# NingZhang1/pyscf_isdf

Measured on AMD Instinct MI355X. Metric: isdf_build_plus_get_jk_wall_time, lower is better.
Workload: dtype f64

## Files before the change

### include/mi355_isdf.h

```cpp
#ifndef MI355_ISDF_H
#define MI355_ISDF_H

#include <stdint.h>

#ifdef __cplusplus
extern "C" {
#endif

typedef struct isdf_ctx* isdf_handle;

#define ISDF_OK 0
#define ISDF_ERR_ARG 1
#define ISDF_ERR_HIP 2
#define ISDF_ERR_LIB 3
#define ISDF_ERR_NUM 4

int isdf_abi_version(void);

int isdf_create(int device_id, isdf_handle* out);
int isdf_destroy(isdf_handle h);
int isdf_set_stream(isdf_handle h, void* hip_stream);
const char* isdf_last_error(isdf_handle h);
int64_t isdf_workspace_bytes(isdf_handle h);
int isdf_release_workspace(isdf_handle h);
// ... 42 lines not shown

int isdf_select_ip(isdf_handle h, const double* d_ao, int nao, int64_t ld,
                   int nblk, const int64_t* blk_off, const int32_t* nip,
                   double tol, double tie_rtol,
                   double* d_L, int64_t ldL, int64_t* d_piv, int32_t* rank);

int isdf_select_ip_ws(isdf_handle h, const double* d_ao, int nao, int64_t ld,
                      int nblk, const int64_t* blk_off, const int32_t* nip,
                      double tol, double tie_rtol,
                      double* d_L, int64_t ldL, int64_t* d_piv, int32_t* rank,
                      void* d_work, int64_t work_bytes);
int64_t isdf_select_ip_work_bytes(int nao, int64_t m);

int isdf_select_ip_gram(isdf_handle h, double* d_A, int m, int64_t ldA, int nip, double tol, double tie_rtol,
                        int panel, int64_t* d_piv, int32_t* rank);

int isdf_select_ip_cplx(isdf_handle h, const double* d_ao, int nao, int nh, int64_t ld,
                        int nblk, const int64_t* blk_off, const int32_t* nip,
                        double tol, double tie_rtol,
                        double* d_L, int64_t ldL, int64_t* d_piv, int32_t* rank);

int isdf_fit_from_chol(isdf_handle h, double* d_L, int k, int64_t m, int64_t ldL,
                       const int64_t* d_piv);

int isdf_fit_prepare(isdf_handle h, const double* d_ao, int nao, int64_t ld,
                     const int64_t* d_ip, int P, double reg_rel, double* d_aoP, double* d_chol,
                     double* reg_used);
int isdf_fit_apply(isdf_handle h, const double* d_chol, const double* d_aoP, int P, int nao,
                   const double* d_ao, int64_t ng, int64_t ld, int forward_only,
                   double* d_theta, int64_t ldt);
int isdf_fit_prepare_cplx(isdf_handle h, const double* d_ao, int nao, int nh, int64_t ld,
                          const int64_t* d_ip, int P, double reg_rel, double* d_aoP, double* d_chol,
                          double* reg_used);
int isdf_fit_apply_cplx(isdf_handle h, const double* d_chol, const double* d_aoP, int P, int nao, int nh,
                        const double* d_ao, int64_t ng, int64_t ld, int forward_only,
                        double* d_theta, int64_t ldt);
int isdf_fit_global(isdf_handle h, const double* d_ao, int nao, int64_t ngrids, int64_t ld,
                    const int64_t* d_ip, int P, double reg_rel, double* d_theta, int64_t ldt,
                    double* d_aoP, double* reg_used);

int isdf_gather_aoP(isdf_handle h, const double* d_ao, int nao, int64_t ld, const int64_t* d_ip, int P,
                    double* d_aoP);
int isdf_gram_sq(isdf_handle h, const double* d_aoP, int P, int nao, int nh, double* d_A);
int isdf_pair_gram_rows(isdf_handle h, const double* d_aoP, int P, int nao, int nh, const double* d_ao,
                        int64_t ng, int64_t ld, double* d_B, int64_t ldb);
int isdf_block_chol(isdf_handle h, const double* d_A, int P, int nblk, const int32_t* blk_off,
                    double shift_rel, double* d_D, double* shift_used);
int isdf_block_solve(isdf_handle h, const double* d_D, int P, int nblk, const int32_t* blk_off, int side,
                     int trans, double* d_X, int64_t n, int64_t ldx);
int isdf_block_invert(isdf_handle h, const double* d_D, int P, int nblk, const int32_t* blk_off, double* d_Dinv);
int isdf_block_apply(isdf_handle h, const double* d_Dinv, int64_t ldd, int nblk, const int32_t* blk_off,
                     double* d_X, int64_t n, int64_t ldx);
int isdf_pair_rows_block_apply(isdf_handle h, const double* d_aoP, int P, int nao, const double* d_ao, int64_t ng,
                               int64_t ld, const double* d_Dinv, int64_t ldd, int nblk, const int32_t* blk_off,
                               double* d_B, int64_t ldb);

int isdf_gram_prod(isdf_handle h, const double* d_aoP, int P, int nao, const double* d_psiP, int nocc, double* d_A);
int isdf_pair_prod_rows(isdf_handle h, const double* d_aoP, int P, int nao, const double* d_psiP, int nocc,
// ... 134 lines not shown
```

### pyscf_isdf_amd/backend.py

```python
import ctypes
import os
import numpy as np
import torch
from . import lib as _lib

_vp = ctypes.c_void_p


def _np_ptr(a):
    return a.ctypes.data_as(_vp)


class HipBackend:
    name = 'hip-gfx950'

    def __init__(self, device=0):
        if not torch.cuda.is_available():
            raise _lib.IsdfError('no GPU visible to torch; the ISDF path has no CPU fallback')
        self.device = torch.device('cuda', device)
        torch.cuda.set_device(self.device)
        self.handle = _lib.Handle(device)
        if os.environ.get('ISDF_TRSM') == 'subst':
            self.set_option('trsm_substitution', 1)
        if os.environ.get('ISDF_OWN_FFT') in ('0', '1', '2'):
# ... 175 lines not shown
        assert piv.dtype == torch.int64 and piv.is_contiguous() and ao.stride(1) == 1 and L.stride(1) == 1
        assert work is None or work.is_contiguous()
        self.handle.call('isdf_select_ip_ws', self._p(ao), ao.shape[0], ao.stride(0), len(nip), _np_ptr(blk_off),
                         _np_ptr(nip), float(tol), float(tie_rtol), self._p(L), L.stride(0), self._p(piv), _np_ptr(rank),
                         None if work is None else self._p(work), 0 if work is None else work.numel() * work.element_size())
        return rank

    def select_ip_gram(self, A, nip, tol, tie_rtol, piv, panel=0):
        self._stream()
        assert piv.dtype == torch.int64 and piv.is_contiguous() and A.stride(1) == 1 and A.shape[0] == A.shape[1]
        rank = ctypes.c_int32(0)
        self.handle.call('isdf_select_ip_gram', self._p(A), A.shape[0], A.stride(0), int(nip), float(tol), float(tie_rtol),
                         int(panel), self._p(piv), ctypes.byref(rank))
        return int(rank.value)

    def fit_from_chol(self, L, k, m, piv):
        self._stream()
        self.handle.call('isdf_fit_from_chol', self._p(L), int(k), int(m), L.stride(0), self._p(piv))

    def fit_prepare(self, ao, ip, reg_rel, aoP, chol):
        self._stream()
        assert ip.dtype == torch.int64 and aoP.is_contiguous() and chol.is_contiguous()
        reg = ctypes.c_double(0.0)
        self.handle.call('isdf_fit_prepare', self._p(ao), ao.shape[0], ao.stride(0), self._p(ip), ip.numel(),
                         float(reg_rel), self._p(aoP), self._p(chol), ctypes.byref(reg))
        return reg.value

    def fit_apply(self, chol, aoP, ao, ng, theta, forward_only=False):
        self._stream()
        self.handle.call('isdf_fit_apply', self._p(chol), self._p(aoP), aoP.shape[0], aoP.shape[1], self._p(ao),
                         int(ng), ao.stride(0), int(bool(forward_only)), self._p(theta), theta.stride(0))

    def gather_aoP(self, ao, ip, aoP):
        self._stream()
        self.handle.call('isdf_gather_aoP', self._p(ao), ao.shape[0], ao.stride(0), self._p(ip), ip.numel(), self._p(aoP))

    def gram_sq(self, aoP, A, nh=0):
        self._stream()
        self.handle.call('isdf_gram_sq', self._p(aoP), aoP.shape[0], aoP.shape[1], int(nh), self._p(A))

    def pair_gram_rows(self, aoP, ao, ng, B, nh=0):
        self._stream()
        self.handle.call('isdf_pair_gram_rows', self._p(aoP), aoP.shape[0], aoP.shape[1], int(nh), self._p(ao), int(ng),
                         ao.stride(0), self._p(B), B.stride(0))

    def gram_prod(self, aoP, psiP, A):
        self._stream()
        assert aoP.is_contiguous() and psiP.is_contiguous() and A.is_contiguous() and aoP.shape[0] == psiP.shape[0]
        self.handle.call('isdf_gram_prod', self._p(aoP), aoP.shape[0], aoP.shape[1], self._p(psiP), psiP.shape[1], self._p(A))

    def pair_prod_rows(self, aoP, psiP, ao, psi, ng, B):
        self._stream()
        assert aoP.is_contiguous() and psiP.is_contiguous() and aoP.shape[0] == psiP.shape[0]
# ... 471 lines not shown
```

### pyscf_isdf_amd/csrc/common.h

```cpp
#pragma once
#include <hip/hip_runtime.h>
#include <rocblas/rocblas.h>
#include <rocsolver/rocsolver.h>
#include <hipfft/hipfft.h>
#include <cstdint>
#include <cstdio>
#include <cstring>
#include <string>
#include <vector>
#include <map>
#include "../../include/mi355_isdf.h"

struct FftPlan {
  hipfftHandle fwd = 0, bwd = 0;
  size_t work_bytes = 0;
};

struct ProfRec {
  hipEvent_t e0 = nullptr, e1 = nullptr;
};
struct ProfEntry {
  std::vector<ProfRec> recs;
  double work = 0.0;
  double ms = 0.0;
// ... 9 lines not shown
};

struct isdf_ctx {
  int profiling = 0;
  std::map<std::string, ProfEntry> prof;
  int device = 0;
  hipStream_t stream = nullptr;
  rocblas_handle blas = nullptr;
  std::string err;
  std::map<std::vector<int>, FftPlan> plans;
  std::map<std::string, std::pair<void*, size_t>> ws;
  int num_cu = 256;
  int trsm_substitution = 0;
  int own_fft = 2;
  int gemm_nn_own = 0;
  int attr_gemm_b = 0, attr_gemm_nn = 0, attr_gram_tri = 0, attr_herm = 0;
  int cand_gram = 1;
  int conv_pipe = 1;
  int conv_sub_rows = 0;
  int gram_pivot_tpb = 256;
  int gram_compact = 1;
  int gram_compact_permille = 875;
  int block_apply_waves = 16;
  int block_apply_reg = 1;
  double coul_omega = 0.0;
  double coul_rc = 0.0;
  int coul_sphere = 0;
  WsKernel wsk;
};

int isdf_fail(isdf_handle h, int code, const char* fmt, ...);
void* isdf_ws(isdf_handle h, const char* name, size_t bytes);
int isdf_get_plan(isdf_handle h, const int32_t mesh[3], int batch, FftPlan** out);
int get_coulG_half(isdf_handle h, const int32_t mesh[3], const double a[9], double extra_scale, double** out);
bool conv_rows_own_supported(const int32_t mesh[3], int nb);
bool conv_rows_q_own_supported(isdf_handle h, const int32_t mesh[3], int nb);
bool spectral_rows_own_supported(isdf_handle h, const int32_t mesh[3], int nb);
// ... 71 lines not shown
                           int64_t ldb);
int gemm_nn_f64(isdf_handle h, int64_t M, int64_t N, int64_t K, const double* A, int64_t lda, const double* B, int64_t ldb,
                double* C, int64_t ldc, bool square);
int gemm_rm(isdf_handle h, char opA, char opB, int64_t M, int64_t N, int64_t K, double alpha,
            const double* A, int64_t lda, const double* B, int64_t ldb, double beta, double* C,
            int64_t ldc);

__host__ __device__ inline int64_t gram_tri_row(int64_t r) {
  const int64_t tm = r >> 8;
  return 32768 * tm * (tm + 1) + (r & 255) * ((tm + 1) << 8);
}
static inline int64_t gram_tri_size(int64_t m) { return m > 0 ? gram_tri_row(m - 1) + (((m - 1) >> 8) + 1) * 256 : 0; }
struct GramTriUnit { int blk, tm, tn, pad; };
int gram_tri_blocks(isdf_handle h, const double* X, int64_t ldx, int K, const GramTriUnit* d_units, int64_t nunits,
                    const int64_t* d_blk_off, int64_t row0, const int64_t* d_tri_off, double* S, double flop);
```

### pyscf_isdf_amd/csrc/fit.hip

```cpp
#include "common.h"
#include <cstdlib>

namespace {

__global__ void gather_T_kernel(const double* __restrict__ L, int64_t ldL,
                                const int64_t* __restrict__ piv, int k, double* __restrict__ T) {
  const int s = blockIdx.x * blockDim.x + threadIdx.x;
  const int t = blockIdx.y;
  if (s >= k) return;
  T[(int64_t)t * k + s] = (s >= t) ? L[(int64_t)t * ldL + piv[s]] : 0.0;
}

__global__ void square_kernel(double* __restrict__ x, int64_t rows, int64_t cols, int64_t ld) {
  const int64_t c = (int64_t)blockIdx.x * blockDim.x + threadIdx.x;
  const int64_t r = blockIdx.y;
  if (c >= cols) return;
  const double v = x[r * ld + c];
  x[r * ld + c] = v * v;
}

__global__ void square_add_kernel(double* __restrict__ x, int64_t ld, const double* __restrict__ y, int64_t ldy,
                                  int64_t cols) {
  const int64_t c = (int64_t)blockIdx.x * blockDim.x + threadIdx.x;
  const int64_t r = blockIdx.y;
// ... 217 lines not shown
  if (nh > 0) {
    double* rot = (double*)isdf_ws(h, "fit_rot", sizeof(double) * (size_t)P * nao);
    double* tmp = (double*)isdf_ws(h, "fit_tmp", sizeof(double) * (size_t)P * P);
    if (!rot || !tmp) return ISDF_ERR_HIP;
    hipLaunchKernelGGL(rotate_kernel, dim3((unsigned)cdiv(nao, 256), (unsigned)P), dim3(256), 0, h->stream, d_aoP, P, nh, rot);
    rc = gemm_rm(h, 'N', 'T', P, P, nao, 1.0, rot, nao, d_aoP, nao, 0.0, tmp, P);
    if (rc) return rc;
    hipLaunchKernelGGL(square_add_kernel, dim3((unsigned)cdiv(P, 256), (unsigned)P), dim3(256), 0, h->stream, d_A,
                       (int64_t)P, tmp, (int64_t)P, (int64_t)P);
  } else {
    hipLaunchKernelGGL(square_kernel, dim3((unsigned)cdiv(P, 256), (unsigned)P), dim3(256), 0, h->stream, d_A,
                       (int64_t)P, (int64_t)P, (int64_t)P);
  }
  KERNEL_CHECK(h);
  return ISDF_OK;
}

extern "C" int isdf_pair_gram_rows(isdf_handle h, const double* d_aoP, int P, int nao, int nh, const double* d_ao,
                                   int64_t ng, int64_t ld, double* d_B, int64_t ldb) {
  if (!h) return ISDF_ERR_ARG;
  ARG_CHECK(h, d_aoP && d_ao && d_B && P > 0 && P <= 65535 && nao > 0 && ng > 0 && ld >= ng && ldb >= ng);
  ARG_CHECK(h, nh == 0 || 2 * nh == nao);
  int rc = product_rows(h, P, ng, nao, d_aoP, d_ao, ld, d_B, ldb, nh == 0);
  if (rc) return rc;
  if (nh > 0) {
    const int64_t CH = 8192;
    double* rot = (double*)isdf_ws(h, "fit_rot", sizeof(double) * (size_t)P * nao);
    double* tmp = (double*)isdf_ws(h, "fit_tmpB", sizeof(double) * (size_t)P * CH);
    if (!rot || !tmp) return ISDF_ERR_HIP;
    hipLaunchKernelGGL(rotate_kernel, dim3((unsigned)cdiv(nao, 256), (unsigned)P), dim3(256), 0, h->stream, d_aoP, P, nh, rot);
// ... 414 lines not shown
```

### pyscf_isdf_amd/csrc/gemm_f64.hip

```cpp
#include "common.h"
#include <cstdlib>

int gemm_rm(isdf_handle h, char opA, char opB, int64_t M, int64_t N, int64_t K, double alpha,
            const double* A, int64_t lda, const double* B, int64_t ldb, double beta, double* C,
            int64_t ldc) {
  ARG_CHECK(h, M < 2147483647LL && N < 2147483647LL && K < 2147483647LL && lda < 2147483647LL &&
                   ldb < 2147483647LL && ldc < 2147483647LL);
  const rocblas_operation ta = (opA == 'N') ? rocblas_operation_none : rocblas_operation_transpose;
  const rocblas_operation tb = (opB == 'N') ? rocblas_operation_none : rocblas_operation_transpose;
  ProfScope ps(h, "rocblas_dgemm[flop]", 2.0 * M * N * (double)K);
  BLAS_TRY(h, rocblas_dgemm(h->blas, tb, ta, (rocblas_int)N, (rocblas_int)M, (rocblas_int)K, &alpha, B,
                            (rocblas_int)ldb, A, (rocblas_int)lda, &beta, C, (rocblas_int)ldc));
  return ISDF_OK;
}

namespace {

typedef double d4 __attribute__((ext_vector_type(4)));

constexpr int BM = 128, BN = 128, BK = 16;
constexpr int LDT = 17;
constexpr int TPB = 256;

struct GemmArgs {
// ... 166 lines not shown
  GemmArgs g;
  g.A = g.B = t.X + (r0 - t.row0) * t.ldx;
  g.lda = g.ldb = t.ldx;
  g.kscale = nullptr;
  g.M = g.N = (int)(t.blk_off[u.blk + 1] - r0);
  g.K = g.kslab = t.K;
  g.ldp = (int64_t)(u.tm + 1) * BM2;
  g.P = t.S + t.tri_off[u.blk] + (gram_tri_row((int64_t)u.tm * BM2) - (int64_t)u.tm * BM2 * g.ldp);
  g.slab_stride = 0;
  g.direct = 1; g.alpha = 1.0; g.beta = 0.0;
  constexpr bool SCALED = false;
  double* sA = smem;
  double* sB = smem + 2 * BM2 * LDT;
  const int tm = u.tm, tn = u.tn, slab = 0;
#include "gemm_nt_b_unit.inc"
}

constexpr int TPBD = 256;

template <bool SCALED>
__global__ __launch_bounds__(TPBD, 2) void gemm_nt_mfma_kernel_d(GemmArgs g) {
  __shared__ double sB[2][BN * LDT];
  const int64_t bid = blockIdx.x;
  const int64_t per_xcd = g.nunits_pad / 8;
  const int64_t unit = (bid % 8) * per_xcd + bid / 8;
  if (unit >= g.nunits) return;
  const int tm = (int)(unit % g.ntm);
  const int tn = (int)((unit / g.ntm) % g.ntn);
  const int slab = (int)(unit / ((int64_t)g.ntm * g.ntn));
  const int64_t k0 = (int64_t)slab * g.kslab;
// ... 576 lines not shown
  GramTriArgs t;
  t.X = X; t.ldx = ldx; t.K = K; t.units = d_units; t.blk_off = d_blk_off; t.row0 = row0; t.tri_off = d_tri_off; t.S = S;
  t.nunits = nunits; t.nunits_pad = cdiv(nunits, 8) * 8;
  ARG_CHECK(h, t.nunits_pad < 2147483647LL);
  const size_t lds = sizeof(double) * 2 * (BM2 + BN) * LDT;
  if (!h->attr_gram_tri) {
    HIP_TRY(h, hipFuncSetAttribute((const void*)gram_tri_mfma_kernel, hipFuncAttributeMaxDynamicSharedMemorySize, (int)lds));
    h->attr_gram_tri = 1;
  }
  ProfScope ps(h, "cand_gram_blocks[flop]", flop);
  hipLaunchKernelGGL(gram_tri_mfma_kernel, dim3((unsigned)t.nunits_pad), dim3(TPB2), lds, h->stream, t);
  KERNEL_CHECK(h);
  return ISDF_OK;
}

bool gemm_nn_f64_supported(isdf_handle h, int64_t M, int64_t N, int64_t K, const double* A, int64_t lda, const double* B,
                           int64_t ldb) {
  return h->gemm_nn_own && M > BM && (double)(cdiv(M, BM2) * BM2) <= 1.15 * (double)M && N >= 2 && N % 2 == 0 && K >= 32 && K % 32 == 0 &&
         lda % 2 == 0 && ldb % 2 == 0 && ((uintptr_t)A) % 16 == 0 && ((uintptr_t)B) % 16 == 0 && M < 2147483647LL &&
         N < 2147483647LL && K < 2147483647LL;
}

int gemm_nn_f64(isdf_handle h, int64_t M, int64_t N, int64_t K, const double* A, int64_t lda, const double* B, int64_t ldb,
                double* C, int64_t ldc, bool square) {
  ARG_CHECK(h, A && B && C && lda >= K && ldb >= N && ldc >= N && gemm_nn_f64_supported(h, M, N, K, A, lda, B, ldb));
  GemmNNArgs g;
  g.A = A; g.lda = lda; g.B = B; g.ldb = ldb; g.C = C; g.ldc = ldc;
  g.M = (int)M; g.N = (int)N; g.K = (int)K;
  g.ntm = (int)cdiv(M, BM2); g.ntn = (int)cdiv(N, BN);
  g.stm = g.ntm >= 4 ? 4 : (g.ntm >= 2 ? 2 : 1);
// ... 18 lines not shown
```

### pyscf_isdf_amd/csrc/gemm_nt_b_unit.inc

```
  const int64_t k0 = (int64_t)slab * g.kslab;
  const int64_t k1 = (k0 + g.kslab < g.K) ? k0 + g.kslab : g.K;
  const int nchunks = (int)((k1 - k0) / BK);
  const int last = nchunks - 1;

  const int tid = threadIdx.x;
  const int lane = tid & 63, wave = tid >> 6;
  const int wm = wave >> 1, wn = wave & 1;
  const int srow = tid >> 3;
  const int sseg = tid & 7;
  const int mlast = g.M - 1, nlast = g.N - 1;
  const double* pA0 = g.A + (int64_t)min(tm * BM2 + srow, mlast) * g.lda + k0 + sseg * 2;
  const double* pA1 = g.A + (int64_t)min(tm * BM2 + srow + 64, mlast) * g.lda + k0 + sseg * 2;
  const double* pA2 = g.A + (int64_t)min(tm * BM2 + srow + 128, mlast) * g.lda + k0 + sseg * 2;
  const double* pA3 = g.A + (int64_t)min(tm * BM2 + srow + 192, mlast) * g.lda + k0 + sseg * 2;
  const double* pB0 = g.B + (int64_t)min(tn * BN + srow, nlast) * g.ldb + k0 + sseg * 2;
  const double* pB1 = g.B + (int64_t)min(tn * BN + srow + 64, nlast) * g.ldb + k0 + sseg * 2;
  const double* pS = SCALED ? g.kscale + k0 + sseg * 2 : nullptr;

  double2 xa0, xa1, xa2, xa3, xb0, xb1, ya0, ya1, ya2, ya3, yb0, yb1;
#define ISDF_LOADB(C, A0, A1, A2, A3, B0, B1)                                                 \
  {                                                                                           \
    const int off = (C) * BK;                                                                 \
    A0 = *reinterpret_cast<const double2*>(pA0 + off);                                        \
    A1 = *reinterpret_cast<const double2*>(pA1 + off);                                        \
// ... 4 lines not shown
    if (SCALED) {                                                                             \
      const double2 sc = *reinterpret_cast<const double2*>(pS + off);                         \
      B0.x *= sc.x; B0.y *= sc.y; B1.x *= sc.x; B1.y *= sc.y;                                 \
    }                                                                                         \
  }
#define ISDF_ST1(P, R) { double* q_ = (P); q_[0] = R.x; q_[1] = R.y; }
#define ISDF_STOREB(BUF, A0, A1, A2, A3, B0, B1)                                              \
  {                                                                                           \
    double* qa = sA + (BUF) * BM2 * LDT + srow * LDT + sseg * 2;                              \
    double* qb = sB + (BUF) * BN * LDT + srow * LDT + sseg * 2;                               \
    ISDF_ST1(qa, A0) ISDF_ST1(qa + 64 * LDT, A1) ISDF_ST1(qa + 128 * LDT, A2)                 \
    ISDF_ST1(qa + 192 * LDT, A3) ISDF_ST1(qb, B0) ISDF_ST1(qb + 64 * LDT, B1)                 \
  }

  d4 acc[4][4];
#pragma unroll
  for (int i = 0; i < 4; ++i)
#pragma unroll
    for (int j = 0; j < 4; ++j) acc[i][j] = (d4){0.0, 0.0, 0.0, 0.0};
  const int frow = lane & 15, fk = lane >> 4;

#define ISDF_FRAGB(KK, AF, BF)                                                                \
    _Pragma("unroll") for (int i = 0; i < 4; ++i) {                                           \
      AF[i] = pa[i * 16 * LDT + (KK) * 4];                                                    \
      BF[i] = pb[i * 16 * LDT + (KK) * 4];                                                    \
    }
#define ISDF_MFMAB(AF, BF)                                                                    \
    _Pragma("unroll") for (int i = 0; i < 4; ++i)                                             \
      _Pragma("unroll") for (int j = 0; j < 4; ++j)                                           \
        acc[i][j] = __builtin_amdgcn_mfma_f64_16x16x4f64(AF[i], BF[j], acc[i][j], 0, 0, 0);
#define ISDF_INTERLEAVE() _Pragma("unroll") for (int q_ = 0; q_ < 8; ++q_) {                  \
    __builtin_amdgcn_sched_group_barrier(0x008, 2, 0); __builtin_amdgcn_sched_group_barrier(0x100, 1, 0); }
#define ISDF_INTERLEAVE_W() _Pragma("unroll") for (int q_ = 0; q_ < 6; ++q_) {                \
    __builtin_amdgcn_sched_group_barrier(0x008, 2, 0); __builtin_amdgcn_sched_group_barrier(0x200, 1, 0); }
// ... 48 lines not shown
    ISDF_CHUNKB(1, ISDF_LOADB(min(c + 3, last), ya0, ya1, ya2, ya3, yb0, yb1), ISDF_STOREB(0, xa0, xa1, xa2, xa3, xb0, xb1))
  }

  double* out = g.P + (int64_t)slab * g.slab_stride;
#pragma unroll
  for (int i = 0; i < 4; ++i) {
#pragma unroll
    for (int r = 0; r < 4; ++r) {
      const int row = tm * BM2 + wm * 64 + i * 16 + (lane >> 4) + 4 * r;
      if (row >= g.M) continue;
#pragma unroll
      for (int j = 0; j < 4; ++j) {
        const int col = tn * BN + wn * 64 + j * 16 + (lane & 15);
        if (col >= g.N) continue;
        double* q = out + (int64_t)row * g.ldp + col;
        const double v = acc[i][j][r];
        if (g.direct) *q = (g.beta == 0.0) ? g.alpha * v : g.alpha * v + g.beta * (*q);
        else *q = v;
      }
    }
  }
```

### pyscf_isdf_amd/csrc/handle.hip

```cpp
#include "common.h"
#include <cstdarg>

int isdf_fail(isdf_handle h, int code, const char* fmt, ...) {
  char buf[1024];
  va_list ap;
  va_start(ap, fmt);
  vsnprintf(buf, sizeof(buf), fmt, ap);
  va_end(ap);
  if (h) h->err = buf;
  else fprintf(stderr, "mi355_isdf: %s\n", buf);
  return code;
}

void* isdf_ws(isdf_handle h, const char* name, size_t bytes) {
  auto& slot = h->ws[name];
  if (slot.second >= bytes && slot.first) return slot.first;
  if (slot.first) {
    (void)hipStreamSynchronize(h->stream);
    (void)hipFree(slot.first);
    slot.first = nullptr;
    slot.second = 0;
  }
  void* p = nullptr;
  hipError_t e = hipMalloc(&p, bytes ? bytes : 8);
// ... 72 lines not shown
  if (std::string(key) == "coul_sphere") { h->coul_sphere = value < 0 ? 0 : value; return ISDF_OK; }
  if (std::string(key) == "conv_pipe") { h->conv_pipe = value != 0; return ISDF_OK; }
  if (std::string(key) == "conv_sub_rows") { h->conv_sub_rows = value < 0 ? 0 : value; return ISDF_OK; }
  if (std::string(key) == "gram_pivot_tpb") {
    if (value != 64 && value != 128 && value != 256) return ISDF_ERR_ARG;
    h->gram_pivot_tpb = value;
    return ISDF_OK;
  }
  if (std::string(key) == "cand_gram") { h->cand_gram = value ? 1 : 0; return ISDF_OK; }
  if (std::string(key) == "gram_compact") { h->gram_compact = value ? 1 : 0; return ISDF_OK; }
  if (std::string(key) == "gram_compact_permille") {
    if (value < 1 || value > 1000) return isdf_fail(h, ISDF_ERR_ARG, "isdf_set_option: gram_compact_permille %d not in [1, 1000]", value);
    h->gram_compact_permille = value;
    return ISDF_OK;
  }
  if (std::string(key) == "block_apply_waves") { h->block_apply_waves = value < 1 ? 1 : value; return ISDF_OK; }
  if (std::string(key) == "block_apply_reg") { h->block_apply_reg = value ? 1 : 0; return ISDF_OK; }
  return isdf_fail(h, ISDF_ERR_ARG, "isdf_set_option: unknown key '%s'", key);
}

int isdf_create(int device_id, isdf_handle* out) {
  if (!out) return ISDF_ERR_ARG;
  *out = nullptr;
  int ndev = 0;
  hipError_t e = hipGetDeviceCount(&ndev);
  if (e != hipSuccess || ndev == 0)
    return isdf_fail(nullptr, ISDF_ERR_HIP, "no HIP device visible (%s)", hipGetErrorString(e));
  if (device_id < 0 || device_id >= ndev)
    return isdf_fail(nullptr, ISDF_ERR_ARG, "device %d out of range (%d devices)", device_id, ndev);
  isdf_ctx* h = new isdf_ctx();
// ... 93 lines not shown
```

### pyscf_isdf_amd/csrc/select_gram.hip

```cpp
#include "common.h"
#include <cfloat>
#include <climits>

namespace {

constexpr int PANEL_MAX = 256;
constexpr int SW = 2048;

struct GramState {
  double tol;
  int rank;
  int done;
};

__device__ inline double wmax(double v) {
  for (int o = 32; o > 0; o >>= 1) v = fmax(v, __shfl_xor(v, o));
  return v;
}
__device__ inline int wmin(int v) {
  for (int o = 32; o > 0; o >>= 1) {
    int u = __shfl_xor(v, o);
    v = u < v ? u : v;
  }
  return v;
// ... 142 lines not shown
  double mx = wmax(valid ? fmax(dnew, 0.0) : 0.0);
  if ((tid & 63) == 0) s_red[tid >> 6] = mx;
  __syncthreads();
  if (tid == 0) {
#pragma unroll
    for (int w = 1; w < NW; ++w) mx = fmax(mx, s_red[w]);
    wg_new[wg] = mx;
    if (wg == 0) {
      piv[j] = p;
      st->rank = j + 1;
      if (j == 0) st->tol = tol;
    }
  }
}

template <int TPB>
__global__ __launch_bounds__(TPB) void gram_compact_diag_kernel(const double* __restrict__ d_src, const int32_t* __restrict__ map,
                                                               int mc, double* __restrict__ d_dst, double* __restrict__ wgmax) {
  __shared__ double red[TPB / 64];
  const int i = blockIdx.x * TPB + threadIdx.x;
  double v = 0.0;
  if (i < mc) {
    v = d_src[map[i]];
    d_dst[i] = v;
  }
  double mx = wmax(i < mc ? fmax(v, 0.0) : 0.0);
  if ((threadIdx.x & 63) == 0) red[threadIdx.x >> 6] = mx;
  __syncthreads();
  if (threadIdx.x == 0) {
    for (int w = 1; w < TPB / 64; ++w) mx = fmax(mx, red[w]);
// ... 23 lines not shown
  const int r = r0 + blockIdx.y;
  const int i = blockIdx.x * 256 + threadIdx.x;
  const int ncol = min(mc, (r / SW + 1) * SW);
  if (i >= ncol) return;
  A[(int64_t)r * ldA + i] = S[(int64_t)blockIdx.y * lds + i];
}

}

namespace {
struct DeviceBuffer {
  void* p = nullptr;
  ~DeviceBuffer() { if (p) (void)hipFree(p); }
};
constexpr int COMPACT_ROWS = 512;
}

extern "C" int isdf_select_ip_gram(isdf_handle h, double* d_A, int m, int64_t ldA, int nip, double tol,
                                   double tie_rtol, int panel, int64_t* d_piv, int32_t* rank) {
  if (!h) return ISDF_ERR_ARG;
  ARG_CHECK(h, d_A && d_piv && rank);
  ARG_CHECK(h, m > 0 && ldA >= m && nip > 0 && tie_rtol >= 0.0 && tie_rtol < 1.0);
  if (panel <= 0) panel = 256;
  ARG_CHECK(h, panel <= PANEL_MAX);
  if (nip > m) nip = m;
  const int TPB = h->gram_pivot_tpb;
  int nwg = (int)cdiv(m, TPB);
  const int64_t ldL = ((int64_t)m + 31) / 32 * 32;
  auto al = [](size_t x) { return (x + 255) / 256 * 256; };
  const size_t b_d = al(sizeof(double) * m), b_w = al(sizeof(double) * nwg), b_st = al(sizeof(GramState));
  const size_t b_L = al(sizeof(double) * (size_t)panel * ldL), b_map = al(sizeof(int32_t) * m);
  char* ws = (char*)isdf_ws(h, "select_gram", 2 * b_d + 2 * b_w + b_st + b_L + 3 * b_map);
  if (!ws) return ISDF_ERR_HIP;
  double* d_d[2];
  double* d_w[2];
  d_d[0] = (double*)ws; ws += b_d;
  d_d[1] = (double*)ws; ws += b_d;
  d_w[0] = (double*)ws; ws += b_w;
  d_w[1] = (double*)ws; ws += b_w;
  GramState* d_st = (GramState*)ws; ws += b_st;
  double* d_Lp = (double*)ws; ws += b_L;
  int32_t* d_map = (int32_t*)ws; ws += b_map;
  int32_t* d_cmap[2];
  d_cmap[0] = (int32_t*)ws; ws += b_map;
  d_cmap[1] = (int32_t*)ws;
  HIP_TRY(h, hipMemsetAsync(d_st, 0, sizeof(GramState), h->stream));
  HIP_TRY(h, hipMemsetAsync(d_piv, 0xff, sizeof(int64_t) * (size_t)nip, h->stream));
  if (TPB == 64) hipLaunchKernelGGL(gram_diag_kernel<64>, dim3(nwg), dim3(64), 0, h->stream, d_A, ldA, m, d_d[0], d_w[0]);
  else if (TPB == 128) hipLaunchKernelGGL(gram_diag_kernel<128>, dim3(nwg), dim3(128), 0, h->stream, d_A, ldA, m, d_d[0], d_w[0]);
  else hipLaunchKernelGGL(gram_diag_kernel<256>, dim3(nwg), dim3(256), 0, h->stream, d_A, ldA, m, d_d[0], d_w[0]);
  KERNEL_CHECK(h);
  int ms = m;
  int rank_at_compact = 0;
  int cc = -1;
  auto piv_to_original = [&](int j1) -> int {
    if (cc < 0 || j1 <= rank_at_compact) return ISDF_OK;
    hipLaunchKernelGGL(gram_piv_to_original_kernel, dim3((unsigned)cdiv(j1 - rank_at_compact, 256)), dim3(256), 0, h->stream,
                       d_piv, rank_at_compact, j1, (const int32_t*)d_cmap[cc]);
    KERNEL_CHECK(h);
    return ISDF_OK;
// ... 33 lines not shown
      for (int i = 0; i < ms; ++i)
        if (!(d_h[i] < 0.0)) map_h.push_back(i);
      mc = (int)map_h.size();
      if (mc > 0 && mc < ms && !stage.p) {
        stage_ld = ((int64_t)mc + 31) / 32 * 32;
        if (hipMalloc(&stage.p, sizeof(double) * (size_t)COMPACT_ROWS * stage_ld) != hipSuccess) {
          (void)hipGetLastError();
          stage.p = nullptr;
          fprintf(stderr, "mi355_isdf: isdf_select_ip_gram: no device memory for the compaction's staging rows (%zu bytes); "
                          "the pick goes on over the whole matrix\n", sizeof(double) * (size_t)COMPACT_ROWS * stage_ld);
          compact = false;
          mc = ms;
        }
      }
    }
    for (int c0 = 0; c0 < ms; c0 += SW) {
      const int c1 = c0 + SW < ms ? c0 + SW : ms;
      int rc = gemm_rm(h, 'T', 'N', ms - c0, c1 - c0, nb, -1.0, d_Lp + c0, ldL, d_Lp + c0, ldL, 1.0,
                       d_A + (int64_t)c0 * ldA + c0, ldA);
      if (rc != ISDF_OK) return rc;
    }
    if (mc == 0 || mc == ms) continue;
    std::vector<int32_t> cm(mc);
    for (int i = 0; i < mc; ++i) cm[i] = cmap_h.empty() ? map_h[i] : cmap_h[map_h[i]];
    cmap_h.swap(cm);
    int rc = piv_to_original(hst.rank);
    if (rc) return rc;
    cc = cc < 0 ? 0 : cc ^ 1;
    HIP_TRY(h, hipMemcpyAsync(d_map, map_h.data(), sizeof(int32_t) * mc, hipMemcpyHostToDevice, h->stream));
    HIP_TRY(h, hipMemcpyAsync(d_cmap[cc], cmap_h.data(), sizeof(int32_t) * mc, hipMemcpyHostToDevice, h->stream));
    {
      ProfScope ps(h, "gram_compact[byte]", 32.0 * 0.5 * (double)mc * mc, 1);
      const int nwc = (int)cdiv(mc, TPB);
      if (TPB == 64) hipLaunchKernelGGL(gram_compact_diag_kernel<64>, dim3(nwc), dim3(64), 0, h->stream, d_d[cur], d_map, mc, d_d[cur ^ 1], d_w[cur ^ 1]);
// ... 29 lines not shown
```

### pyscf_isdf_amd/isdf.py

```python
import os
import sys
import time
import warnings
import numpy as np
import torch
from . import gto
from ._common import (UniformGrids, partition_grid_by_atom, _monkhorst_pack_size, _aoslice_by_atom,
                      _default_fft_batch)
from .fit_route import FitRouteMixin
from .sharded import ShardedMixin
from .kpoints import KPointMixin
from .hcore import HcoreMixin
from .eri_surface import EriSurfaceMixin


class ISDF(FitRouteMixin, ShardedMixin, KPointMixin, HcoreMixin, EriSurfaceMixin):
    _keys = {'cell', 'kpts', 'grids', 'mesh', 'blockdim', 'exxdiv', 'c_isdf', 'select', 'tie_rtol'}

    def __init__(self, cell, kpts=np.zeros((1, 3)), c_isdf=12, select='refined', backend=None, comm=None):
        self.cell = cell
        self.stdout = getattr(cell, 'stdout', None) or sys.stdout
        self.verbose = getattr(cell, 'verbose', 0)
        self.max_memory = getattr(cell, 'max_memory', 4000)
        self.kpts_symm = None
# ... 5 lines not shown
        self.blockdim = 240
        self.exxdiv = None
        self.c_isdf = c_isdf
        self.select = select
        self.refine_over = 2.0
        self.pair_space = 'ao'
        self.occ_refit = 'always'
        self.w_spectral = True
        self.w_sphere = 'auto'
        self.w_sphere_tol = 1e-11
        self.w_sort_bins = 256
        self.w_spectral_check_tol = 5e-9
        self.w_spectral_max_c = 18
        self.cand_skip_zero_rows = True
        self.cand_gram = True
        self.cand_ao_cutoff = None
        self.tie_rtol = 1e-10
        self.select_tol = -1.0
        self.reg_rel = 1e-12
        self.reg_used = 0.0
        self.k_ip_factor = None
        self.kpt_pair_q = 'auto'
        self.kpt_w_spectral = False
        self.kpts_band = None
        self.force_sharded = False
        self.fit_route = 'auto'
        self.bj_check_tol = 3e-8
        self.bj_auto_kpts = False
        self.bj_max_c = 12
        self.bj_nprobe = 8
# ... 567 lines not shown
        del aoC, gram, psiC
        own = owner[chosen]
        self._refined_by_atom = [chosen[own == b] for b in range(natm)]
        return np.array([len(x) for x in self._refined_by_atom], dtype=np.int32)

    def _refine_pick(self, aoC, cand, P_target, gram=None, nh=0, psiC=None):
        be = self.backend
        m = len(cand)
        P_target = min(int(P_target), m)
        A = be.empty((m, m)) if gram is None else gram
        if psiC is not None and nh:
            be.gram_prod_cplx(aoC, nh, psiC, psiC.shape[1] // 2, A)
        elif psiC is not None:
            be.gram_prod(aoC, psiC, A)
        else:
            be.gram_sq(aoC, A, nh)
        piv2 = be.empty((P_target,), dtype=torch.int64)
        r2 = be.select_ip_gram(A, P_target, self.select_tol, self.tie_rtol, piv2)
        chosen = np.asarray(cand)[be.to_host(piv2)[:r2]]
        del A, piv2
        return chosen

    def _keep_V_for_robust_k(self, t0):
        if not self.robust_k:
            return
        be = self.backend
        theta = self._fit_state['theta']
        mesh = np.asarray(self.mesh, dtype=np.int32)
        a = np.asarray(self.cell.lattice_vectors(), dtype=float)
        be.coulomb_rows(theta, mesh, a, self._last_fft_batch)
        self._V = theta
# ... 340 lines not shown
```

### pyscf_isdf_amd/lib.py

```python
import ctypes
import os

_HERE = os.path.dirname(os.path.abspath(__file__))
LIB_PATH = os.path.join(_HERE, 'lib', 'libmi355_isdf.so')
ABI_VERSION = 21

_lib = None

c_int, c_i64, c_dbl, c_vp = ctypes.c_int, ctypes.c_int64, ctypes.c_double, ctypes.c_void_p

SIGNATURES = {
    'isdf_abi_version': (c_int, []),
    'isdf_create': (c_int, [c_int, ctypes.POINTER(c_vp)]),
    'isdf_destroy': (c_int, [c_vp]),
    'isdf_set_stream': (c_int, [c_vp, c_vp]),
    'isdf_last_error': (ctypes.c_char_p, [c_vp]),
    'isdf_workspace_bytes': (c_i64, [c_vp]),
    'isdf_set_coulomb_omega': (c_int, [c_vp, c_dbl]),
    'isdf_set_coulomb_cutoff': (c_int, [c_vp, c_dbl]),
    'isdf_set_coulomb_ws': (c_int, [c_vp, c_dbl, c_vp, c_vp, c_vp, c_vp]),
    'isdf_set_option': (c_int, [c_vp, ctypes.c_char_p, c_int]),
    'isdf_release_workspace': (c_int, [c_vp]),
    'isdf_prof_enable': (c_int, [c_vp, c_int]),
    'isdf_prof_reset': (c_int, [c_vp]),
    'isdf_prof_count': (c_int, [c_vp]),
    'isdf_prof_get': (c_int, [c_vp, c_int, ctypes.c_char_p, c_int, ctypes.POINTER(c_i64), ctypes.POINTER(c_dbl), ctypes.POINTER(c_dbl)]),
    'isdf_eval_ao': (c_int, [c_vp, c_vp, c_int, c_vp, c_int, c_vp, c_int, c_vp, c_int, c_vp, c_vp, c_i64, c_vp, c_i64]),
    'isdf_block_row_absmax': (c_int, [c_vp, c_vp, c_int, c_i64, c_int, c_vp, c_vp]),
    'isdf_gather_cols': (c_int, [c_vp, c_vp, c_int, c_i64, c_vp, c_i64, c_vp, c_i64]),
    'isdf_partition_by_atom': (c_int, [c_vp, c_vp, c_i64, c_vp, c_int, c_vp, c_dbl, c_vp]),
    'isdf_select_ip': (c_int, [c_vp, c_vp, c_int, c_i64, c_int, c_vp, c_vp, c_dbl, c_dbl, c_vp, c_i64, c_vp, c_vp]),
    'isdf_select_ip_ws': (c_int, [c_vp, c_vp, c_int, c_i64, c_int, c_vp, c_vp, c_dbl, c_dbl, c_vp, c_i64, c_vp, c_vp, c_vp,
                                  c_i64]),
    'isdf_select_ip_work_bytes': (c_i64, [c_int, c_i64]),
    'isdf_select_ip_gram': (c_int, [c_vp, c_vp, c_int, c_i64, c_int, c_dbl, c_dbl, c_int, c_vp, ctypes.POINTER(ctypes.c_int32)]),
    'isdf_fit_from_chol': (c_int, [c_vp, c_vp, c_int, c_i64, c_i64, c_vp]),
    'isdf_fit_prepare': (c_int, [c_vp, c_vp, c_int, c_i64, c_vp, c_int, c_dbl, c_vp, c_vp, ctypes.POINTER(c_dbl)]),
    'isdf_fit_apply': (c_int, [c_vp, c_vp, c_vp, c_int, c_int, c_vp, c_i64, c_i64, c_int, c_vp, c_i64]),
    'isdf_gather_aoP': (c_int, [c_vp, c_vp, c_int, c_i64, c_vp, c_int, c_vp]),
    'isdf_gram_sq': (c_int, [c_vp, c_vp, c_int, c_int, c_int, c_vp]),
    'isdf_pair_gram_rows': (c_int, [c_vp, c_vp, c_int, c_int, c_int, c_vp, c_i64, c_i64, c_vp, c_i64]),
    'isdf_gram_prod': (c_int, [c_vp, c_vp, c_int, c_int, c_vp, c_int, c_vp]),
    'isdf_pair_prod_rows': (c_int, [c_vp, c_vp, c_int, c_int, c_vp, c_int, c_vp, c_i64, c_vp, c_i64, c_i64, c_vp, c_i64]),
    'isdf_factor_solve_half': (c_int, [c_vp, c_vp, c_int, c_int, c_vp, c_i64, c_i64]),
    'isdf_gram_prod_cplx': (c_int, [c_vp, c_vp, c_int, c_int, c_int, c_vp, c_int, c_int, c_vp]),
    'isdf_pair_prod_rows_cplx': (c_int, [c_vp, c_vp, c_int, c_int, c_int, c_vp, c_int, c_int, c_vp, c_i64, c_vp, c_i64, c_i64,
                                         c_vp, c_i64]),
    'isdf_block_chol': (c_int, [c_vp, c_vp, c_int, c_int, c_vp, c_dbl, c_vp, ctypes.POINTER(c_dbl)]),
    'isdf_block_solve': (c_int, [c_vp, c_vp, c_int, c_int, c_vp, c_int, c_int, c_vp, c_i64, c_i64]),
    'isdf_block_invert': (c_int, [c_vp, c_vp, c_int, c_int, c_vp, c_vp]),
    'isdf_block_apply': (c_int, [c_vp, c_vp, c_i64, c_int, c_vp, c_vp, c_i64, c_i64]),
    'isdf_pair_rows_block_apply': (c_int, [c_vp, c_vp, c_int, c_int, c_vp, c_i64, c_i64, c_vp, c_i64, c_int, c_vp, c_vp, c_i64]),
    'isdf_shift_diag': (c_int, [c_vp, c_vp, c_int, c_dbl]),
    'isdf_chol_inplace': (c_int, [c_vp, c_vp, c_int, c_dbl, c_vp, ctypes.POINTER(c_dbl)]),
    'isdf_factor_solve': (c_int, [c_vp, c_vp, c_int, c_vp, c_i64, c_i64]),
# ... 117 lines not shown
```

Baseline: 16.96.

## Add lower-triangular MFMA kernel for Gram build and pivoted-Cholesky trailing update

```diff
diff --git a/include/mi355_isdf.h b/include/mi355_isdf.h
--- a/include/mi355_isdf.h
+++ b/include/mi355_isdf.h
@@ -80,6 +80,7 @@
 
 int isdf_select_ip_gram(isdf_handle h, double* d_A, int m, int64_t ldA, int nip, double tol, double tie_rtol,
                         int panel, int64_t* d_piv, int32_t* rank);
+int isdf_gram_trailing_update(isdf_handle h, double* d_A, int ms, int64_t ldA, const double* d_Lp, int64_t ldL, int nb);
 
 int isdf_select_ip_cplx(isdf_handle h, const double* d_ao, int nao, int nh, int64_t ld,
                         int nblk, const int64_t* blk_off, const int32_t* nip,
@@ -108,6 +109,7 @@
 int isdf_gather_aoP(isdf_handle h, const double* d_ao, int nao, int64_t ld, const int64_t* d_ip, int P,
                     double* d_aoP);
 int isdf_gram_sq(isdf_handle h, const double* d_aoP, int P, int nao, int nh, double* d_A);
+int isdf_gram_sq_lower(isdf_handle h, const double* d_aoP, int P, int nao, int nh, double* d_A, int64_t ldA);
 int isdf_pair_gram_rows(isdf_handle h, const double* d_aoP, int P, int nao, int nh, const double* d_ao,
                         int64_t ng, int64_t ld, double* d_B, int64_t ldb);
 int isdf_block_chol(isdf_handle h, const double* d_A, int P, int nblk, const int32_t* blk_off,
diff --git a/pyscf_isdf_amd/backend.py b/pyscf_isdf_amd/backend.py
--- a/pyscf_isdf_amd/backend.py
+++ b/pyscf_isdf_amd/backend.py
@@ -213,6 +213,11 @@
                          int(panel), self._p(piv), ctypes.byref(rank))
         return int(rank.value)
 
+    def gram_trailing_update(self, A, Lp, nb):
+        self._stream()
+        assert A.stride(1) == 1 and Lp.stride(1) == 1 and A.shape[0] == A.shape[1] and Lp.shape[1] >= A.shape[0]
+        self.handle.call('isdf_gram_trailing_update', self._p(A), A.shape[0], A.stride(0), self._p(Lp), Lp.stride(0), int(nb))
+
     def fit_from_chol(self, L, k, m, piv):
         self._stream()
         self.handle.call('isdf_fit_from_chol', self._p(L), int(k), int(m), L.stride(0), self._p(piv))
@@ -234,8 +239,14 @@
         self._stream()
         self.handle.call('isdf_gather_aoP', self._p(ao), ao.shape[0], ao.stride(0), self._p(ip), ip.numel(), self._p(aoP))
 
-    def gram_sq(self, aoP, A, nh=0):
-        self._stream()
+    has_gram_sq_lower = True
+
+    def gram_sq(self, aoP, A, nh=0, lower=False):
+        self._stream()
+        if lower:
+            assert aoP.is_contiguous() and A.stride(1) == 1
+            self.handle.call('isdf_gram_sq_lower', self._p(aoP), aoP.shape[0], aoP.shape[1], int(nh), self._p(A), A.stride(0))
+            return
         self.handle.call('isdf_gram_sq', self._p(aoP), aoP.shape[0], aoP.shape[1], int(nh), self._p(A))
 
     def pair_gram_rows(self, aoP, ao, ng, B, nh=0):
diff --git a/pyscf_isdf_amd/csrc/common.h b/pyscf_isdf_amd/csrc/common.h
--- a/pyscf_isdf_amd/csrc/common.h
+++ b/pyscf_isdf_amd/csrc/common.h
@@ -47,13 +47,14 @@
   int trsm_substitution = 0;
   int own_fft = 2;
   int gemm_nn_own = 0;
-  int attr_gemm_b = 0, attr_gemm_nn = 0, attr_gram_tri = 0, attr_herm = 0;
+  int attr_gemm_b = 0, attr_gemm_nn = 0, attr_gram_tri = 0, attr_herm = 0, attr_gram_lower = 0;
   int cand_gram = 1;
   int conv_pipe = 1;
   int conv_sub_rows = 0;
   int gram_pivot_tpb = 256;
   int gram_compact = 1;
   int gram_compact_permille = 875;
+  int gram_update_own = 1;
   int block_apply_waves = 16;
   int block_apply_reg = 1;
   double coul_omega = 0.0;
@@ -155,3 +156,13 @@
 struct GramTriUnit { int blk, tm, tn, pad; };
 int gram_tri_blocks(isdf_handle h, const double* X, int64_t ldx, int K, const GramTriUnit* d_units, int64_t nunits,
                     const int64_t* d_blk_off, int64_t row0, const int64_t* d_tri_off, double* S, double flop);
+
+constexpr int GRAM_STRIP = 2048;
+struct GramLowerUnit { int tm, tn; };
+int gram_lower_units_upload(isdf_handle h, int m, const GramLowerUnit** d_units, int64_t* nunits);
+double gram_lower_entries(int m);
+bool gram_lower_supported(const double* X, int64_t ld, int K);
+int gram_update_lower(isdf_handle h, const double* negLT, const double* LT, int64_t kpad, int nb, double* C, int64_t ldc, int m,
+                      const GramLowerUnit* d_units, int64_t nunits);
+int gram_sq_lower(isdf_handle h, const double* X, int64_t ldx, int K, double* C, int64_t ldc, int m, const GramLowerUnit* d_units,
+                  int64_t nunits);
diff --git a/pyscf_isdf_amd/csrc/fit.hip b/pyscf_isdf_amd/csrc/fit.hip
--- a/pyscf_isdf_amd/csrc/fit.hip
+++ b/pyscf_isdf_amd/csrc/fit.hip
@@ -255,6 +255,20 @@
   }
   KERNEL_CHECK(h);
   return ISDF_OK;
+}
+
+extern "C" int isdf_gram_sq_lower(isdf_handle h, const double* d_aoP, int P, int nao, int nh, double* d_A, int64_t ldA) {
+  if (!h) return ISDF_ERR_ARG;
+  ARG_CHECK(h, d_aoP && d_A && P > 0 && nao > 0 && P <= 65535 && ldA >= P && (nh == 0 || 2 * nh == nao));
+  if (nh != 0 || !gram_lower_supported(d_aoP, nao, nao)) {
+    ARG_CHECK(h, ldA == P);
+    return isdf_gram_sq(h, d_aoP, P, nao, nh, d_A);
+  }
+  const GramLowerUnit* d_units = nullptr;
+  int64_t nunits = 0;
+  int rc = gram_lower_units_upload(h, P, &d_units, &nunits);
+  if (rc) return rc;
+  return gram_sq_lower(h, d_aoP, nao, nao, d_A, ldA, P, d_units, nunits);
 }
 
 extern "C" int isdf_pair_gram_rows(isdf_handle h, const double* d_aoP, int P, int nao, int nh, const double* d_ao,
diff --git a/pyscf_isdf_amd/csrc/gemm_f64.hip b/pyscf_isdf_amd/csrc/gemm_f64.hip
--- a/pyscf_isdf_amd/csrc/gemm_f64.hip
+++ b/pyscf_isdf_amd/csrc/gemm_f64.hip
@@ -204,6 +204,52 @@
   double* sB = smem + 2 * BM2 * LDT;
   const int tm = u.tm, tn = u.tn, slab = 0;
 #include "gemm_nt_b_unit.inc"
+}
+
+struct GramLowerArgs {
+  const double* A; const double* B; int64_t ld; int K;
+  double* C; int64_t ldc; int m;
+  const GramLowerUnit* units;
+  int64_t nunits, nunits_pad;
+};
+
+template <bool UPDATE>
+__global__ __launch_bounds__(TPB2, 2) void gram_lower_mfma_kernel(GramLowerArgs t) {
+  extern __shared__ double smem[];
+  const int64_t bid = blockIdx.x;
+  const int64_t per_xcd = t.nunits_pad / 8;
+  const int64_t unit = (bid % 8) * per_xcd + bid / 8;
+  if (unit >= t.nunits) return;
+  const GramLowerUnit u = t.units[unit];
+  GemmArgs g;
+  g.A = t.A; g.B = t.B;
+  g.lda = g.ldb = t.ld;
+  g.kscale = nullptr;
+  g.M = g.N = t.m;
+  g.K = g.kslab = t.K;
+  g.P = t.C; g.ldp = t.ldc;
+  g.slab_stride = 0;
+  g.direct = 1; g.alpha = 1.0; g.beta = 0.0;
+  constexpr bool SCALED = false;
+  double* sA = smem;
+  double* sB = smem + 2 * BM2 * LDT;
+  const int tm = u.tm, tn = u.tn, slab = 0;
+  if constexpr (UPDATE) {
+#define ISDF_UNIT_ACC_INIT                                                                    \
+  _Pragma("unroll") for (int i = 0; i < 4; ++i)                                               \
+    _Pragma("unroll") for (int r = 0; r < 4; ++r) {                                           \
+      const int row = tm * BM2 + wm * 64 + i * 16 + (lane >> 4) + 4 * r;                      \
+      const double* crow = g.P + (int64_t)min(row, mlast) * g.ldp;                            \
+      _Pragma("unroll") for (int j = 0; j < 4; ++j) {                                         \
+        const int col = tn * BN + wn * 64 + j * 16 + (lane & 15);                             \
+        acc[i][j][r] = crow[min(col, nlast)];                                                 \
+      }                                                                                       \
+    }
+#include "gemm_nt_b_unit.inc"
+  } else {
+#define ISDF_UNIT_OUT(v) ((v) * (v))
+#include "gemm_nt_b_unit.inc"
+  }
 }
 
 constexpr int TPBD = 256;
@@ -810,6 +856,74 @@
   return ISDF_OK;
 }
 
+static void gram_lower_units(int m, std::vector<GramLowerUnit>& out) {
+  out.clear();
+  const int ntm = (int)cdiv(m, BM2), ntn = (int)cdiv(m, BN);
+  constexpr int TS = GRAM_STRIP / BN;
+  for (int tn0 = 0; tn0 < ntn; tn0 += TS) {
+    const int tm0 = (int)((int64_t)tn0 * BN / BM2);
+    for (int a = tm0; a < ntm; a += 8)
+      for (int b = tn0; b < std::min(tn0 + TS, ntn); b += 4)
+        for (int tn = b; tn < std::min(std::min(b + 4, tn0 + TS), ntn); ++tn)
+          for (int tm = a; tm < std::min(a + 8, ntm); ++tm) out.push_back(GramLowerUnit{tm, tn});
+  }
+}
+
+int gram_lower_units_upload(isdf_handle h, int m, const GramLowerUnit** d_units, int64_t* nunits) {
+  std::vector<GramLowerUnit> units;
+  gram_lower_units(m, units);
+  void* d = isdf_ws(h, "gram_lower_units", sizeof(GramLowerUnit) * units.size());
+  if (!d) return ISDF_ERR_HIP;
+  HIP_TRY(h, hipMemcpyAsync(d, units.data(), sizeof(GramLowerUnit) * units.size(), hipMemcpyHostToDevice, h->stream));
+  HIP_TRY(h, hipStreamSynchronize(h->stream));
+  *d_units = (const GramLowerUnit*)d;
+  *nunits = (int64_t)units.size();
+  return ISDF_OK;
+}
+
+double gram_lower_entries(int m) {
+  double n = 0.0;
+  for (int c0 = 0; c0 < m; c0 += GRAM_STRIP) n += (double)(m - c0) * (double)std::min(GRAM_STRIP, m - c0);
+  return n;
+}
+
+bool gram_lower_supported(const double* X, int64_t ld, int K) {
+  return K > 0 && K % 32 == 0 && ld >= K && ld % 2 == 0 && ((uintptr_t)X) % 16 == 0;
+}
+
+static int gram_lower_launch(isdf_handle h, bool update, const double* A, const double* B, int64_t ld, int K, double* C,
+                             int64_t ldc, int m, const GramLowerUnit* d_units, int64_t nunits, const char* label, double flop) {
+  ARG_CHECK(h, A && B && C && d_units && nunits > 0 && m > 0 && ldc >= m && gram_lower_supported(A, ld, K) &&
+                   gram_lower_supported(B, ld, K));
+  GramLowerArgs t;
+  t.A = A; t.B = B; t.ld = ld; t.K = K; t.C = C; t.ldc = ldc; t.m = m; t.units = d_units;
+  t.nunits = nunits; t.nunits_pad = cdiv(nunits, 8) * 8;
+  ARG_CHECK(h, t.nunits_pad < 2147483647LL);
+  const size_t lds = sizeof(double) * 2 * (BM2 + BN) * LDT;
+  if (!h->attr_gram_lower) {
+    HIP_TRY(h, hipFuncSetAttribute((const void*)gram_lower_mfma_kernel<true>, hipFuncAttributeMaxDynamicSharedMemorySize, (int)lds));
+    HIP_TRY(h, hipFuncSetAttribute((const void*)gram_lower_mfma_kernel<false>, hipFuncAttributeMaxDynamicSharedMemorySize, (int)lds));
+    h->attr_gram_lower = 1;
+  }
+  ProfScope ps(h, label, flop);
+  if (update) hipLaunchKernelGGL(gram_lower_mfma_kernel<true>, dim3((unsigned)t.nunits_pad), dim3(TPB2), lds, h->stream, t);
+  else hipLaunchKernelGGL(gram_lower_mfma_kernel<false>, dim3((unsigned)t.nunits_pad), dim3(TPB2), lds, h->stream, t);
+  KERNEL_CHECK(h);
+  return ISDF_OK;
+}
+
+int gram_update_lower(isdf_handle h, const double* negLT, const double* LT, int64_t kpad, int nb, double* C, int64_t ldc, int m,
+                      const GramLowerUnit* d_units, int64_t nunits) {
+  return gram_lower_launch(h, true, negLT, LT, kpad, (int)kpad, C, ldc, m, d_units, nunits, "gram_update_lower[flop]",
+                           2.0 * nb * gram_lower_entries(m));
+}
+
+int gram_sq_lower(isdf_handle h, const double* X, int64_t ldx, int K, double* C, int64_t ldc, int m, const GramLowerUnit* d_units,
+                  int64_t nunits) {
+  return gram_lower_launch(h, false, X, X, ldx, K, C, ldc, m, d_units, nunits, "gram_sq_lower[flop]",
+                           2.0 * K * gram_lower_entries(m));
+}
+
 bool gemm_nn_f64_supported(isdf_handle h, int64_t M, int64_t N, int64_t K, const double* A, int64_t lda, const double* B,
                            int64_t ldb) {
   return h->gemm_nn_own && M > BM && (double)(cdiv(M, BM2) * BM2) <= 1.15 * (double)M && N >= 2 && N % 2 == 0 && K >= 32 && K % 32 == 0 &&
diff --git a/pyscf_isdf_amd/csrc/gemm_nt_b_unit.inc b/pyscf_isdf_amd/csrc/gemm_nt_b_unit.inc
--- a/pyscf_isdf_amd/csrc/gemm_nt_b_unit.inc
+++ b/pyscf_isdf_amd/csrc/gemm_nt_b_unit.inc
@@ -1,3 +1,11 @@
+#ifndef ISDF_UNIT_ACC_INIT
+#define ISDF_UNIT_ACC_INIT                                                                    \
+  _Pragma("unroll") for (int i = 0; i < 4; ++i)                                               \
+    _Pragma("unroll") for (int j = 0; j < 4; ++j) acc[i][j] = (d4){0.0, 0.0, 0.0, 0.0};
+#endif
+#ifndef ISDF_UNIT_OUT
+#define ISDF_UNIT_OUT(v) (v)
+#endif
   const int64_t k0 = (int64_t)slab * g.kslab;
   const int64_t k1 = (k0 + g.kslab < g.K) ? k0 + g.kslab : g.K;
   const int nchunks = (int)((k1 - k0) / BK);
@@ -42,10 +50,7 @@
   }
 
   d4 acc[4][4];
-#pragma unroll
-  for (int i = 0; i < 4; ++i)
-#pragma unroll
-    for (int j = 0; j < 4; ++j) acc[i][j] = (d4){0.0, 0.0, 0.0, 0.0};
+  ISDF_UNIT_ACC_INIT
   const int frow = lane & 15, fk = lane >> 4;
 
 #define ISDF_FRAGB(KK, AF, BF)                                                                \
@@ -124,9 +129,11 @@
         const int col = tn * BN + wn * 64 + j * 16 + (lane & 15);
         if (col >= g.N) continue;
         double* q = out + (int64_t)row * g.ldp + col;
-        const double v = acc[i][j][r];
+        const double v = ISDF_UNIT_OUT(acc[i][j][r]);
         if (g.direct) *q = (g.beta == 0.0) ? g.alpha * v : g.alpha * v + g.beta * (*q);
         else *q = v;
       }
     }
   }
+#undef ISDF_UNIT_ACC_INIT
+#undef ISDF_UNIT_OUT
diff --git a/pyscf_isdf_amd/csrc/handle.hip b/pyscf_isdf_amd/csrc/handle.hip
--- a/pyscf_isdf_amd/csrc/handle.hip
+++ b/pyscf_isdf_amd/csrc/handle.hip
@@ -110,6 +110,7 @@
     h->gram_compact_permille = value;
     return ISDF_OK;
   }
+  if (std::string(key) == "gram_update_own") { h->gram_update_own = value ? 1 : 0; return ISDF_OK; }
   if (std::string(key) == "block_apply_waves") { h->block_apply_waves = value < 1 ? 1 : value; return ISDF_OK; }
   if (std::string(key) == "block_apply_reg") { h->block_apply_reg = value ? 1 : 0; return ISDF_OK; }
   return isdf_fail(h, ISDF_ERR_ARG, "isdf_set_option: unknown key '%s'", key);
diff --git a/pyscf_isdf_amd/csrc/select_gram.hip b/pyscf_isdf_amd/csrc/select_gram.hip
--- a/pyscf_isdf_amd/csrc/select_gram.hip
+++ b/pyscf_isdf_amd/csrc/select_gram.hip
@@ -5,7 +5,7 @@
 namespace {
 
 constexpr int PANEL_MAX = 256;
-constexpr int SW = 2048;
+constexpr int SW = GRAM_STRIP;
 
 struct GramState {
   double tol;
@@ -180,6 +180,28 @@
   }
 }
 
+__global__ __launch_bounds__(256) void gram_panel_transpose_kernel(const double* __restrict__ Lp, int64_t ldL, int nb, int ms,
+                                                                   int kpad, double* __restrict__ LT, double* __restrict__ negLT) {
+  __shared__ double tile[32][33];
+  const int tx = threadIdx.x & 31, ty = threadIdx.x >> 5;
+  const int i0 = blockIdx.x * 32, t0 = blockIdx.y * 32;
+#pragma unroll
+  for (int q = 0; q < 4; ++q) {
+    const int t = t0 + ty + 8 * q, i = i0 + tx;
+    tile[ty + 8 * q][tx] = (t < nb && i < ms) ? Lp[(int64_t)t * ldL + i] : 0.0;
+  }
+  __syncthreads();
+#pragma unroll
+  for (int q = 0; q < 4; ++q) {
+    const int i = i0 + ty + 8 * q, t = t0 + tx;
+    if (i < ms) {
+      const double v = tile[tx][ty + 8 * q];
+      LT[(int64_t)i * kpad + t] = v;
+      negLT[(int64_t)i * kpad + t] = -v;
+    }
+  }
+}
+
 template <int TPB>
 __global__ __launch_bounds__(TPB) void gram_compact_diag_kernel(const double* __restrict__ d_src, const int32_t* __restrict__ map,
                                                                int mc, double* __restrict__ d_dst, double* __restrict__ wgmax) {
@@ -233,6 +255,41 @@
   ~DeviceBuffer() { if (p) (void)hipFree(p); }
 };
 constexpr int COMPACT_ROWS = 512;
+}
+
+static int trailing_update(isdf_handle h, bool own, double* d_A, int64_t ldA, int ms, const double* d_Lp, int64_t ldL, int nb,
+                           double* d_LT, double* d_negLT, const GramLowerUnit* d_units, int64_t nunits) {
+  if (own) {
+    const int kpad = (nb + 31) / 32 * 32;
+    hipLaunchKernelGGL(gram_panel_transpose_kernel, dim3((unsigned)cdiv(ms, 32), (unsigned)(kpad / 32)), dim3(256), 0, h->stream,
+                       d_Lp, ldL, nb, ms, kpad, d_LT, d_negLT);
+    KERNEL_CHECK(h);
+    return gram_update_lower(h, d_negLT, d_LT, kpad, nb, d_A, ldA, ms, d_units, nunits);
+  }
+  for (int c0 = 0; c0 < ms; c0 += SW) {
+    const int c1 = c0 + SW < ms ? c0 + SW : ms;
+    int rc = gemm_rm(h, 'T', 'N', ms - c0, c1 - c0, nb, -1.0, d_Lp + c0, ldL, d_Lp + c0, ldL, 1.0,
+                     d_A + (int64_t)c0 * ldA + c0, ldA);
+    if (rc != ISDF_OK) return rc;
+  }
+  return ISDF_OK;
+}
+
+extern "C" int isdf_gram_trailing_update(isdf_handle h, double* d_A, int ms, int64_t ldA, const double* d_Lp, int64_t ldL, int nb) {
+  if (!h) return ISDF_ERR_ARG;
+  ARG_CHECK(h, d_A && d_Lp && ms > 0 && ldA >= ms && ldL >= ms && nb > 0 && nb <= PANEL_MAX);
+  const bool own = h->gram_update_own != 0;
+  double* d_LT = nullptr;
+  const GramLowerUnit* d_units = nullptr;
+  int64_t nunits = 0;
+  const size_t nT = (size_t)ms * (size_t)((nb + 31) / 32 * 32);
+  if (own) {
+    d_LT = (double*)isdf_ws(h, "select_gram_T", sizeof(double) * 2 * nT);
+    if (!d_LT) return ISDF_ERR_HIP;
+    int rc = gram_lower_units_upload(h, ms, &d_units, &nunits);
+    if (rc != ISDF_OK) return rc;
+  }
+  return trailing_update(h, own, d_A, ldA, ms, d_Lp, ldL, nb, d_LT, d_LT + nT, d_units, nunits);
 }
 
 extern "C" int isdf_select_ip_gram(isdf_handle h, double* d_A, int m, int64_t ldA, int nip, double tol,
@@ -249,7 +306,10 @@
   auto al = [](size_t x) { return (x + 255) / 256 * 256; };
   const size_t b_d = al(sizeof(double) * m), b_w = al(sizeof(double) * nwg), b_st = al(sizeof(GramState));
   const size_t b_L = al(sizeof(double) * (size_t)panel * ldL), b_map = al(sizeof(int32_t) * m);
-  char* ws = (char*)isdf_ws(h, "select_gram", 2 * b_d + 2 * b_w + b_st + b_L + 3 * b_map);
+  const bool own_update = h->gram_update_own != 0;
+  const int64_t kpad_max = ((int64_t)panel + 31) / 32 * 32;
+  const size_t b_T = own_update ? al(sizeof(double) * (size_t)m * kpad_max) : 0;
+  char* ws = (char*)isdf_ws(h, "select_gram", 2 * b_d + 2 * b_w + b_st + b_L + 3 * b_map + 2 * b_T);
   if (!ws) return ISDF_ERR_HIP;
   double* d_d[2];
   double* d_w[2];
@@ -262,7 +322,12 @@
   int32_t* d_map = (int32_t*)ws; ws += b_map;
   int32_t* d_cmap[2];
   d_cmap[0] = (int32_t*)ws; ws += b_map;
-  d_cmap[1] = (int32_t*)ws;
+  d_cmap[1] = (int32_t*)ws; ws += b_map;
+  double* d_LT = (double*)ws; ws += b_T;
+  double* d_negLT = (double*)ws;
+  const GramLowerUnit* d_units = nullptr;
+  int64_t nunits = 0;
+  int units_ms = -1;
   HIP_TRY(h, hipMemsetAsync(d_st, 0, sizeof(GramState), h->stream));
   HIP_TRY(h, hipMemsetAsync(d_piv, 0xff, sizeof(int64_t) * (size_t)nip, h->stream));
   if (TPB == 64) hipLaunchKernelGGL(gram_diag_kernel<64>, dim3(nwg), dim3(64), 0, h->stream, d_A, ldA, m, d_d[0], d_w[0]);
@@ -326,10 +391,13 @@
         }
       }
     }
-    for (int c0 = 0; c0 < ms; c0 += SW) {
-      const int c1 = c0 + SW < ms ? c0 + SW : ms;
-      int rc = gemm_rm(h, 'T', 'N', ms - c0, c1 - c0, nb, -1.0, d_Lp + c0, ldL, d_Lp + c0, ldL, 1.0,
-                       d_A + (int64_t)c0 * ldA + c0, ldA);
+    if (own_update && units_ms != ms) {
+      int rc = gram_lower_units_upload(h, ms, &d_units, &nunits);
+      if (rc != ISDF_OK) return rc;
+      units_ms = ms;
+    }
+    {
+      int rc = trailing_update(h, own_update, d_A, ldA, ms, d_Lp, ldL, nb, d_LT, d_negLT, d_units, nunits);
       if (rc != ISDF_OK) return rc;
     }
     if (mc == 0 || mc == ms) continue;
diff --git a/pyscf_isdf_amd/isdf.py b/pyscf_isdf_amd/isdf.py
--- a/pyscf_isdf_amd/isdf.py
+++ b/pyscf_isdf_amd/isdf.py
@@ -43,6 +43,7 @@
         self.w_spectral_max_c = 18
         self.cand_skip_zero_rows = True
         self.cand_gram = True
+        self.gram_lower = True
         self.cand_ao_cutoff = None
         self.tie_rtol = 1e-10
         self.select_tol = -1.0
@@ -640,7 +641,8 @@
         elif psiC is not None:
             be.gram_prod(aoC, psiC, A)
         else:
-            be.gram_sq(aoC, A, nh)
+            kw = {'lower': True} if self.gram_lower and getattr(be, 'has_gram_sq_lower', False) else {}
+            be.gram_sq(aoC, A, nh, **kw)
         piv2 = be.empty((P_target,), dtype=torch.int64)
         r2 = be.select_ip_gram(A, P_target, self.select_tol, self.tie_rtol, piv2)
         chosen = np.asarray(cand)[be.to_host(piv2)[:r2]]
diff --git a/pyscf_isdf_amd/lib.py b/pyscf_isdf_amd/lib.py
--- a/pyscf_isdf_amd/lib.py
+++ b/pyscf_isdf_amd/lib.py
@@ -38,7 +38,9 @@
     'isdf_fit_prepare': (c_int, [c_vp, c_vp, c_int, c_i64, c_vp, c_int, c_dbl, c_vp, c_vp, ctypes.POINTER(c_dbl)]),
     'isdf_fit_apply': (c_int, [c_vp, c_vp, c_vp, c_int, c_int, c_vp, c_i64, c_i64, c_int, c_vp, c_i64]),
     'isdf_gather_aoP': (c_int, [c_vp, c_vp, c_int, c_i64, c_vp, c_int, c_vp]),
+    'isdf_gram_trailing_update': (c_int, [c_vp, c_vp, c_int, c_i64, c_vp, c_i64, c_int]),
     'isdf_gram_sq': (c_int, [c_vp, c_vp, c_int, c_int, c_int, c_vp]),
+    'isdf_gram_sq_lower': (c_int, [c_vp, c_vp, c_int, c_int, c_int, c_vp, c_i64]),
     'isdf_pair_gram_rows': (c_int, [c_vp, c_vp, c_int, c_int, c_int, c_vp, c_i64, c_i64, c_vp, c_i64]),
     'isdf_gram_prod': (c_int, [c_vp, c_vp, c_int, c_int, c_vp, c_int, c_vp]),
     'isdf_pair_prod_rows': (c_int, [c_vp, c_vp, c_int, c_int, c_vp, c_int, c_vp, c_i64, c_vp, c_i64, c_i64, c_vp, c_i64]),
```

Result: no change. 16.81 (median of 6 runs) (-0.9%).
